# tsirigos/ibm-cbc-genomic-tools

Measured on AMD Instinct MI355X. Metric: overlap-counted reads/sec, 100M reads x 1M ref intervals, higher is better.
Workload: dtype int32; 1 GPU; BASELINE config 3: 100000000 50bp reads in total, sorted by (chrom,start), x 1000000 ref intervals over 24 hg38 chromosomes, strand ignored (genomic_overlaps count -S -i); reads resident in HBM; total_reads=100000000, refs=1000000, reduce=none (one rank)

## Files before the change

ibm-cbc-genomic-tools_amd/csrc/gtx_capi.hip:

```cpp
#include <hip/hip_runtime.h>
#include <stdint.h>
#include <string.h>
#include <stdio.h>
#include <algorithm>
#include <string>
#include <thread>
#include <vector>
#include "gtx.h"
#include "gtx_kernels.h"
#include "gtx_pairs.h"
#include "gtx_internal.h"
#include "gtx_ctx.h"

static thread_local std::string g_create_error;

int make_hist_set(gtx_ctx *c, HistSet &h, int64_t histLen)
{
  const size_t parts = (size_t)gtx::scan_tiles(histLen) + 2;
  HIPCHK(c, h.histA.alloc(histLen)); HIPCHK(c, h.histB.alloc(histLen)); HIPCHK(c, h.partA.alloc(parts)); HIPCHK(c, h.partB.alloc(parts));
  HIPCHK(c, h.prefA.alloc(histLen)); HIPCHK(c, h.prefB.alloc(histLen)); HIPCHK(c, h.flags.alloc(8 * parts));
  HIPCHK(c, h.totals.alloc(4 * parts));
  for (DevBuf<u64> *b : {&h.histA, &h.histB, &h.partA, &h.partB, &h.totals}) HIPCHK(c, hipMemset(b->get(), 0, sizeof(u64) * b->cap));
  HIPCHK(c, hipMemset(h.flags.get(), 0, sizeof(unsigned) * h.flags.cap));
  h.epoch = 0; h.draws = 0; h.totalsTurn = 0;
// ... 178 lines not shown
    if (cl > maxc) maxc = cl;
  }
  if (nClasses <= 0) nClasses = maxc + 1;
  if (maxc >= nClasses) return fail(c, GTX_E_RANGE, "gtx_set_refs: class id >= n_classes");
  if (nClasses < 1) nClasses = 1;

  std::vector<u64> keyE, keyS;
  std::vector<int32_t> ord;
  ord.reserve(m);
  const bool keepZero = (flags & GTX_REFS_KEEP_ZERO_LENGTH) != 0;
  for (int64_t k = 0; k < m; k++) {
    int32_t s = tri[3 * k + 1], e = tri[3 * k + 2];
    const bool take = tri[3 * k] >= 0 && (keepZero ? (int64_t)s <= (int64_t)e + 1 : !(s > e || e <= 0));
    if (take) ord.push_back((int32_t)k);
  }
  const int64_t nv = (int64_t)ord.size();
  struct Item { int32_t cls; int32_t val; int32_t k; };
  std::vector<Item> itE(nv), itS(nv);
  for (int64_t i = 0; i < nv; i++) {
    int32_t k = ord[i];
    itE[i] = {tri[3 * (int64_t)k], tri[3 * (int64_t)k + 2], k};
    itS[i] = {tri[3 * (int64_t)k], tri[3 * (int64_t)k + 1], k};
  }
  auto cmp = [](const Item &a, const Item &b) { return a.cls != b.cls ? a.cls < b.cls : (a.val != b.val ? a.val < b.val : a.k < b.k); };
  if (nv > (1 << 16)) {
    std::thread other([&] { std::sort(itS.begin(), itS.end(), cmp); });
    std::sort(itE.begin(), itE.end(), cmp);
    other.join();
  } else {
    std::sort(itE.begin(), itE.end(), cmp);
    std::sort(itS.begin(), itS.end(), cmp);
  }

  std::vector<int32_t> sortedE(nv + 1), sortedS(nv + 1), seg(nClasses + 1, 0), posE(m > 0 ? m : 1, -1), posS(m > 0 ? m : 1, -1), classBase(m > 0 ? m : 1, -1);
  for (int64_t i = 0; i < nv; i++) seg[itE[i].cls + 1]++;
  for (int cl = 0; cl < nClasses; cl++) seg[cl + 1] += seg[cl];
  for (int64_t i = 0; i < nv; i++) {
    sortedE[i] = itE[i].val; posE[itE[i].k] = (int32_t)(i + itE[i].cls);
    sortedS[i] = itS[i].val; posS[itS[i].k] = (int32_t)(i + itS[i].cls);
    classBase[itE[i].k] = seg[itE[i].cls] + itE[i].cls - 1;
  }

  c->nRefs = -1;
  c->ix = {}; c->cv = {}; c->rx = {}; c->share = {};
  c->covDirty = false; c->pairUsed = false;
  const int64_t histLen = nv + nClasses;
  HIPCHK(c, c->ix.sortedE.alloc(nv + 1));
  HIPCHK(c, c->ix.sortedS.alloc(nv + 1));
  HIPCHK(c, c->ix.segStart.alloc(nClasses + 1));
  HIPCHK(c, c->ix.posE.alloc(m + 1));
  HIPCHK(c, c->ix.posS.alloc(m + 1));
  HIPCHK(c, c->ix.classBase.alloc(m + 1));
  { int rc = make_hist_set(c, c->ix.hist, histLen); if (rc) return rc; }
  c->histDirty = false; c->tileSumsValid = true;
  HIPCHK(c, hipMemcpy(c->ix.sortedE.get(), sortedE.data(), sizeof(int32_t) * nv, hipMemcpyHostToDevice));
  HIPCHK(c, hipMemcpy(c->ix.sortedS.get(), sortedS.data(), sizeof(int32_t) * nv, hipMemcpyHostToDevice));
  HIPCHK(c, hipMemcpy(c->ix.segStart.get(), seg.data(), sizeof(int32_t) * (nClasses + 1), hipMemcpyHostToDevice));
  {
    c->ix.sampShift = gtx::search_sample_shift(nv);
    c->ix.nSamp = (int)((nv + (1ll << c->ix.sampShift) - 1) >> c->ix.sampShift);
    std::vector<int32_t> sampE(c->ix.nSamp + 1), sampS(c->ix.nSamp + 1);
    for (int i = 0; i < c->ix.nSamp; i++) { sampE[i] = sortedE[(int64_t)i << c->ix.sampShift]; sampS[i] = sortedS[(int64_t)i << c->ix.sampShift]; }
    HIPCHK(c, upload(c->ix.sampE, sampE.data(), sampE.size()));
    HIPCHK(c, upload(c->ix.sampS, sampS.data(), sampS.size()));
    const int64_t nTop = (nv + 255) >> 8;
    std::vector<int32_t> topE(nTop + 1), topS(nTop + 1);
    for (int64_t i = 0; i < nTop; i++) { topE[i] = sortedE[i << 8]; topS[i] = sortedS[i << 8]; }
    HIPCHK(c, upload(c->ix.topE, topE.data(), topE.size()));
    HIPCHK(c, upload(c->ix.topS, topS.data(), topS.size()));
  }
  { int rc = make_place_table(c, seg, sortedE, sortedS, nClasses, nv, c->ix.place); if (rc) return rc; }
  {
    const int kE = gtx::bucket_e_size(), kS = gtx::bucket_s_size();
    BucketCuts k;
    k.clsStart.assign(nClasses + 1, 0);
    for (int cl = 0; cl < nClasses; cl++) {
      k.clsStart[cl] = (int32_t)k.posHi.size();
      const int32_t s0 = seg[cl], s1 = seg[cl + 1];
      for (int32_t e0 = s0; e0 < s1; e0 += kE) {
        const int32_t e1 = std::min<int64_t>((int64_t)e0 + kE, s1);
        k.posHi.push_back(e1 == s1 ? INT32_MAX : sortedE[e1 - 1]);
        k.eLo.push_back(e0); k.eHi.push_back(e1); k.cls.push_back(cl);
        const int32_t lo = e0 == s0 ? s0 : (int32_t)(std::upper_bound(sortedS.begin() + s0, sortedS.begin() + s1, sortedE[e0 - 1]) - sortedS.begin());
        k.sLo.push_back(lo); k.sHi.push_back((int32_t)std::min<int64_t>((int64_t)lo + kS, s1));
      }
    }
    k.clsStart[nClasses] = (int32_t)k.posHi.size();
    if (k.posHi.size() <= 8192 && nClasses <= 2048) {
      int rc = build_bucket_tables(c, c->ix.bkt, k, nClasses); if (rc) return rc;
    }
  }
  if (m > 0) {
    HIPCHK(c, hipMemcpy(c->ix.posE.get(), posE.data(), sizeof(int32_t) * m, hipMemcpyHostToDevice));
    HIPCHK(c, hipMemcpy(c->ix.posS.get(), posS.data(), sizeof(int32_t) * m, hipMemcpyHostToDevice));
    HIPCHK(c, hipMemcpy(c->ix.classBase.get(), classBase.data(), sizeof(int32_t) * m, hipMemcpyHostToDevice));
  }
  c->h_refS.resize(m > 0 ? m : 1); c->h_refE.resize(m > 0 ? m : 1); c->h_refC.resize(m > 0 ? m : 1);
  for (int64_t k = 0; k < m; k++) { c->h_refC[k] = tri[3 * k]; c->h_refS[k] = tri[3 * k + 1]; c->h_refE[k] = tri[3 * k + 2]; }
  c->mergeRefs = keepZero;
  if (keepZero) {
    std::vector<int4> sp; std::vector<int32_t> spIdx;
    for (int64_t k = 0; k < m; k++)
      if (tri[3 * k] >= 0 && (int64_t)tri[3 * k + 1] > (int64_t)tri[3 * k + 2] + 1) { sp.push_back(make_int4(tri[3 * k], tri[3 * k + 1], tri[3 * k + 2], 0)); spIdx.push_back((int32_t)k); }
    c->rx.nSpecial = (int)sp.size();
    if (c->rx.nSpecial) {
      HIPCHK(c, upload(c->rx.specialRefs, sp.data(), sp.size()));
      HIPCHK(c, upload(c->rx.specialIdx, spIdx.data(), spIdx.size()));
      HIPCHK(c, c->rx.specialOut.alloc(sp.size()));
      HIPCHK(c, hipMemset(c->rx.specialOut.get(), 0, sizeof(u64) * sp.size()));
    }
  }
  c->nRefs = m; c->nValid = nv; c->nClasses = nClasses; c->histLen = histLen;
  c->h_seg = seg;
  return GTX_OK;
}

#ifdef GTX_WAVE_TRACE
static constexpr size_t kTraceWaves = 1u << 20;
static unsigned long long *g_trace = nullptr;
static unsigned long long *gtx_debug_trace_buffer()
{
  if (!g_trace && hipMalloc(&g_trace, kTraceWaves * 32) == hipSuccess) (void)hipMemset(g_trace, 0, kTraceWaves * 32);
  return g_trace;
}
extern "C" int gtx_debug_trace_read(unsigned long long *out, long long nWaves)
{
  if (!g_trace || nWaves > (long long)kTraceWaves) return -1;
  if (hipDeviceSynchronize() != hipSuccess) return -2;
// ... 119 lines not shown
  if (!c->sideUsed) return GTX_OK;
  c->sideUsed = false;
  HIPCHK(c, gtx::launch_side_reads(c->rx.refC.get(), c->rx.refS.get(), c->rx.refE.get(), c->nRefs, c->side.get(), c->sideCount.get(), c->sideCap, c->specialMode, (u64 *)d_out,
                                   c->d_info.get() + c->infoCur, c->stream));
  HIPCHK(c, gtx::launch_special_scatter(c->rx.specialIdx.get(), c->rx.specialOut.get(), c->rx.nSpecial, (u64 *)d_out, c->sideCount.get(), c->stream));
  return GTX_OK;
}

extern "C" {

static int count_begin(gtx_ctx *c)
{
  if (c->histDirty) {
    HistSet &h = c->ix.hist;
    for (DevBuf<u64> *b : {&h.histA, &h.histB, &h.partA, &h.partB, &h.totals}) HIPCHK(c, hipMemsetAsync(b->get(), 0, sizeof(u64) * b->cap, c->stream));
  }
  if (c->histDirty || c->covDirty) HIPCHK(c, hipMemcpyAsync(c->d_info.get() + c->infoCur, &c->h_info.get()[1], sizeof(gtx::DevInfo), hipMemcpyHostToDevice, c->stream));
  if ((c->histDirty || c->covDirty) && c->sideCount.get()) {
    HIPCHK(c, hipMemsetAsync(c->sideCount.get(), 0, sizeof(unsigned), c->stream));
    if (c->rx.nSpecial) HIPCHK(c, hipMemsetAsync(c->rx.specialOut.get(), 0, sizeof(u64) * c->rx.nSpecial, c->stream));
  }
  if (c->histDirty && c->rx.pairAcc.get()) HIPCHK(c, hipMemsetAsync(c->rx.pairAcc.get(), 0, sizeof(u64) * 2 * (size_t)std::max<int64_t>(c->nRefs, 1), c->stream));
  c->sideUsed = false; c->pairUsed = false;
  c->histDirty = true; c->tileSumsValid = true;
  c->ix.lastShareInfo = nullptr;
  return GTX_OK;
}

static int finalize_set(gtx_ctx *c, HistSet &h, bool sumsValid, u64 *d_hits, gtx::DevInfo *info, gtx::DevInfo *infoNext, hipStream_t s,
                        const gtx::FinalizeShare *fs, bool hist32)
{
  if (++h.epoch == 0) { HIPCHK(c, hipMemsetAsync(h.flags.get(), 0, sizeof(unsigned) * h.flags.cap, s)); h.epoch = 1; h.draws = 0; }
  gtx::FinalizeArgs a = h.view(c->histLen);
  a.tileSumsValid = sumsValid; a.localMaxTiles = c->localMaxTiles; a.posE = c->ix.posE.get(); a.posS = c->ix.posS.get(); a.classBase = c->ix.classBase.get();
  a.m = c->nRefs; a.hits = d_hits; a.info = info; a.nextInfo = infoNext; a.share = fs; a.hist32 = hist32;
  gtx::FinalizeRoute took;
  HIPCHK(c, gtx::launch_finalize(a, s, &took));
  if (took == gtx::FIN_CHAINED) h.draws += (unsigned long long)(fs ? fs->nTiles : gtx::scan_tiles(c->histLen));
  if (took == gtx::FIN_LOCAL) h.totalsTurn ^= 1;
  return GTX_OK;
}

static int count_end(gtx_ctx *c, void *d_hits, bool share = false, bool scatter = false, bool hist32 = false)
{
  const gtx::FinalizeShare fs = {c->share.tiles.get(), c->share.nTiles, c->share.regions.get(), c->share.nRegions, scatter};
  int rc = finalize_set(c, c->ix.hist, c->tileSumsValid, (u64 *)d_hits, c->d_info.get() + c->infoCur, c->d_info.get() + (c->infoCur ^ 1), c->stream,
                        share ? &fs : nullptr, hist32);
  if (rc) return rc;
  rc = merge_end(c, d_hits); if (rc) return rc;
  c->histDirty = false;
  c->infoCur ^= 1;
  return GTX_OK;
}

int gtx_count_device(gtx_ctx *c, const void *d_reads, const void *d_weights, int64_t n, uint32_t flags, void *d_hits)
{
  if (!c) return GTX_E_ARG;
  if (c->nRefs < 0) return fail(c, GTX_E_STATE, "gtx_count_device: gtx_set_refs has not been called");
  if (n < 0 || (n > 0 && !d_reads) || (c->nRefs > 0 && !d_hits)) return fail(c, GTX_E_ARG, "gtx_count_device: bad argument");
  HIPCHK(c, hipSetDevice(c->device));
  int rc = count_begin(c); if (rc) return rc;
  prof_begin(c);
  HIPCHK(c, prof_mark(c, 1, c->stream));
  rc = merge_prepare(c, flags, 0); if (rc) return rc;
  const bool streaming = (flags & (GTX_READS_SORTED | GTX_CHECK_SORTED)) != 0;
  if (!streaming) c->tileSumsValid = false;
  bool h32 = false;
// ... 668 lines not shown
```

ibm-cbc-genomic-tools_amd/csrc/gtx_ctx.h:

```cpp
#pragma once
#include <hip/hip_runtime.h>
#include <stdint.h>
#include <string.h>
#include <algorithm>
#include <string>
#include <utility>
#include <vector>
#include "gtx.h"
#include "gtx_kernels.h"
#include "gtx_pairs.h"
#include "gtx_link.h"
#include "gtx_adjacent.h"
#include "gtx_internal.h"

namespace gtx { struct JoinInfo; struct SignalInfo; }

#pragma GCC visibility push(hidden)

typedef unsigned long long u64;

namespace gtxhost {

template <class T, bool Pinned> class Buf {
 public:
// ... 25 lines not shown
  DevBuf<int4> cls; DevBuf<int> rank; int shift = 0;
  gtx::PlaceTable view() const { gtx::PlaceTable t; t.cls = cls.get(); t.rank = rank.get(); t.shift = shift; return t; }
};

struct BucketTables {
  DevBuf<int> bkt; DevBuf<int4> clsCell; DevBuf<uint16_t> cellTab; int nB = 0, nCells = 0, cellShift = 0;
  gtx::BucketTable view() const
  {
    gtx::BucketTable t;
    const int *d = bkt.get();
    t.posHi = d; t.eLo = d + nB; t.eHi = d + 2 * nB; t.sLo = d + 3 * nB; t.sHi = d + 4 * nB; t.cls = d + 5 * nB; t.clsStart = d + 6 * nB; t.nB = nB;
    t.clsCell = clsCell.get(); t.cellTab = cellTab.get(); t.nCells = nCells; t.cellShift = cellShift;
    return t;
  }
};

struct BucketCuts { std::vector<int32_t> posHi, eLo, eHi, sLo, sHi, cls, clsStart; };

struct HistSet {
  DevBuf<u64> histA, histB, partA, partB, prefA, prefB; DevBuf<unsigned> flags; unsigned epoch = 0; unsigned long long draws = 0;
  DevBuf<u64> totals; unsigned totalsTurn = 0;
  gtx::FinalizeArgs view(int64_t histLen) const
  {
    gtx::FinalizeArgs a = {};
    const size_t turn = 2 * ((size_t)gtx::scan_tiles(histLen) + 2);
    a.histA = histA.get(); a.histB = histB.get(); a.tileA = partA.get(); a.tileB = partB.get(); a.prefA = prefA.get(); a.prefB = prefB.get(); a.histLen = histLen;
    a.chainFlags = flags.get(); a.epoch = epoch; a.draws = draws;
    a.totals = totals.get() + (totalsTurn & 1) * turn; a.nextTotals = totals.get() + ((totalsTurn & 1) ^ 1) * turn;
    return a;
  }
};

struct CountIndex {
  DevBuf<int> sortedE, sortedS, segStart, posE, posS, classBase;
  DevBuf<int> sampE, sampS; int sampShift = 6, nSamp = 0;
  DevBuf<int> topE, topS;
  PlaceTable place;
  BucketTables bkt;
  HistSet hist;
  HistSet alt[GTXI_SHARE_STREAMS];
  DevBuf<gtx::DevInfo> info3; unsigned shareSeq = 0; unsigned shareTurn[GTXI_SHARE_STREAMS] = {}; const gtx::DevInfo *lastShareInfo = nullptr;
};

struct CoverIndex {
  DevBuf<u64> cov[12];
  DevBuf<int> sortedT, segT, topT, posTE, posTS, classBaseT;
  int64_t histLenT = 0;
  PlaceTable place;
  BucketTables bkt;
  bool ready = false;
};

struct RefExtras {
  DevBuf<int> refS, refE, refC;
  int nSpecial = 0; DevBuf<int4> specialRefs; DevBuf<int> specialIdx; DevBuf<u64> specialOut;
  struct PairIdx { DevBuf<int> mem; int n = 0; bool built = false; gtx::PairIndex ix = {}; } pairMulti, pairAll;
  DevBuf<int2> blkOf, blkIv; bool refBlocks = false;
  DevBuf<u64> pairAcc;
  DevBuf<long long> joinKey; std::vector<long long> h_joinKey; int joinMono = -1;
  DevBuf<int4> offRef; DevBuf<int8_t> refStrand;
  bool sigSet = false; double sigMin = 0, sigMax = 0; int64_t sigBins = 0; DevBuf<long long> sigRefLen;
};

struct Share { bool on = false; DevBuf<int> tiles; int nTiles = 0; DevBuf<int> regions; int64_t nRegions = 0, offset = 0; DevBuf<unsigned char> owned; };

struct TextSlot {
  DevBuf<char> text; DevBuf<unsigned> seg;
// ... 274 lines not shown
```

ibm-cbc-genomic-tools_amd/csrc/gtx_kernels.h:

```cpp
#pragma once
#include <hip/hip_runtime.h>
#include <stdint.h>
#include <mutex>
#include "gtx_routes.h"

namespace gtx {

struct PerDevice {
  std::mutex m; unsigned long long done = 0;
  template <class F> hipError_t once(F fn)
  {
    int dev = 0;
    hipError_t e = hipGetDevice(&dev);
    if (e != hipSuccess) return e;
    std::lock_guard<std::mutex> lk(m);
    if (dev >= 0 && dev < 64 && ((done >> dev) & 1)) return hipSuccess;
    e = fn();
    if (e == hipSuccess && dev >= 0 && dev < 64) done |= 1ull << dev;
    return e;
  }
};

struct DevInfo {
  long long first_unsorted;
// ... 112 lines not shown
int bucket_e_size();
int bucket_s_size();
int bucket_t_size();
hipError_t launch_count_bucketed(const void *reads, const void *weights, long long n, const CountArgs &a, const BucketTable &t,
                                 const BucketWork &w, const BucketPlan &p, hipStream_t st);
hipError_t launch_cover_bucketed(const void *reads, const void *weights, long long n, const CountArgs &a, const CoverArgs &cv, const BucketTable &t,
                                 const BucketWork &w, const BucketPlan &p, hipStream_t st);
struct ScanPart { int bucket, first, count, pad; };
int scan_part_bins(bool weighted);
hipError_t launch_scan_bucketed(const void *reads, const void *weights, long long n, const CountArgs &a, const ScanArgs &sc, const BucketTable &t,
                                const BucketWork &w, const BucketPlan &p, const ScanPart *parts, int nParts, hipStream_t st,
                                unsigned long long *out = nullptr);
int scan_fused_max_comb();
hipError_t launch_tile_sums(unsigned long long *histA, unsigned long long *histB, long long histLen, unsigned long long *tileA, unsigned long long *tileB, hipStream_t st);

hipError_t launch_special_refs(const void *reads, const void *weights, long long n, const int4 *refs, int nSpecial, int mode,
                               unsigned long long *out, hipStream_t st);
hipError_t launch_side_reads(const int *refC, const int *refS, const int *refE, long long m, const int4 *side, const unsigned *sideCount,
                             int sideCap, int mode, unsigned long long *hits, DevInfo *info, hipStream_t st);
hipError_t launch_special_scatter(const int *specialIdx, unsigned long long *specialOut, int nSpecial, unsigned long long *hits,
                                  unsigned *sideCount, hipStream_t st);

SpanSchedule span_schedule(long long nChunks, int cpw, int r, long long slots);
int search_sample_shift(long long nValid);

hipError_t launch_count(const void *reads, const void *weights, long long n, const CountArgs &a, bool sortedHint, hipStream_t st);
struct FinalizeShare { const int *tileList; int nTiles; const int *regionList; long long nRegions; bool scatter; };
struct FinalizeArgs {
  unsigned long long *histA, *histB, *tileA, *tileB, *prefA, *prefB;
  unsigned *chainFlags; unsigned epoch; unsigned long long draws;
  unsigned long long *totals, *nextTotals;
  long long histLen; bool tileSumsValid;
  int localMaxTiles;
  const int *posE, *posS, *classBase; long long m; unsigned long long *hits;
  DevInfo *info, *nextInfo;
  const FinalizeShare *share; bool hist32;
};
hipError_t launch_finalize(const FinalizeArgs &a, hipStream_t st, FinalizeRoute *took);
hipError_t launch_coverage(const void *reads, const void *weights, long long n, const CoverArgs &a, hipStream_t st);
hipError_t launch_coverage_finalize(const CoverArgs &a, long long histLen, const CoverGather &g, long long m,
                                    unsigned long long *cov, DevInfo *nextInfo, hipStream_t st);
hipError_t launch_scan_zero(void *micro, long long bytes, const int *runIf, hipStream_t st);
hipError_t launch_scan_hist(const void *reads, const void *weights, long long n, const ScanArgs &a, hipStream_t st, const int *runIf = nullptr);
int scan_window_tile();
hipError_t launch_scan_windows(const void *micro, bool micro64, const ScanArgs &a, long long totalTiles,
                               unsigned long long *out, hipStream_t st, const int *runIf = nullptr);

struct ScanOwn {
  const long long *blkOff;
  int tile;
  long long totalBlocks;
  long long *bounds;
  int *flag;
};
int scan_own_tile(long long nReads, long long totalMicro, int comb);
hipError_t launch_scan_own(const void *reads, const void *weights, long long n, const ScanArgs &a, const ScanOwn &o,
                           unsigned long long *out, hipStream_t st);

}
```

ibm-cbc-genomic-tools_amd/csrc/gtx_kernels.hip:

```cpp
#include <hip/hip_runtime.h>
#include <stdint.h>
#include <stdlib.h>
#include <string.h>
#include <stdio.h>
#include <type_traits>
#include <vector>
#include <algorithm>
#include "gtx_kernels.h"

namespace gtx {

typedef unsigned long long u64;
typedef long long i64;

static constexpr int kHi = 0x7fffffff;
static constexpr int kLo = (int)0x80000000;
static constexpr int kSlots = 63;
static constexpr int kSearchLdsBytes = 128 * 1024;

__device__ __forceinline__ int rfl(int v) { return __builtin_amdgcn_readfirstlane(v); }
__device__ __forceinline__ int rdlane(int v, int l) { return __builtin_amdgcn_readlane(v, l); }

__device__ __forceinline__ int lane_prev(int v) { return __builtin_amdgcn_update_dpp(v, v, 0x138, 0xf, 0xf, false); }

// ... 1179 lines not shown
      else if (s0 != s1) {
        const int i0 = (int)(((i64)s0 + rnd) >> sh), i1 = (int)(((i64)s1 + rnd) >> sh);
        int lo = i0, hi = i1;
        while (lo < hi) { int mid = (lo + hi) >> 1; if (se[mid] < t.s) lo = mid + 1; else hi = mid; }
        int glo = lo == i0 ? s0 : ((lo - 1) << sh) + 1, ghi = lo == i1 ? s1 : lo << sh;
        while (glo < ghi) { int mid = (int)(((i64)glo + ghi) >> 1); if (a.sortedE[mid] < t.s) glo = mid + 1; else ghi = mid; }
        slotA = glo + t.c;
        lo = i0; hi = i1;
        while (lo < hi) { int mid = (lo + hi) >> 1; if (ss[mid] <= t.e) lo = mid + 1; else hi = mid; }
        glo = lo == i0 ? s0 : ((lo - 1) << sh) + 1; ghi = lo == i1 ? s1 : lo << sh;
        while (glo < ghi) { int mid = (int)(((i64)glo + ghi) >> 1); if (a.sortedS[mid] <= t.e) glo = mid + 1; else ghi = mid; }
        slotB = glo + t.c;
      }
    }
    if (WEIGHTED) {
      if (slotA >= 0) { atomicAdd(&a.histA[slotA], (u64)w); atomicAdd(&a.histB[slotB], (u64)w); }
    } else {
      run_add(a.histA, slotA, lane);
      run_add(a.histB, slotB, lane);
    }
  }
  if (nNoClass) atomicAdd((u64 *)&a.info->n_no_class, (u64)nNoClass);
  if (nDegen) { atomicAdd((u64 *)&a.info->n_degenerate, (u64)nDegen); atomicMin((i64 *)&a.info->first_degenerate, firstDegen + a.indexBase); }
}

template <class T> __device__ __forceinline__ void load4(const T *p, u64 (&v)[4]);
template <> __device__ __forceinline__ void load4<u64>(const u64 *p, u64 (&v)[4])
{ const ulonglong2 x = *(const ulonglong2 *)p, y = *(const ulonglong2 *)(p + 2); v[0] = x.x; v[1] = x.y; v[2] = y.x; v[3] = y.y; }
template <> __device__ __forceinline__ void load4<unsigned>(const unsigned *p, u64 (&v)[4])
{ const uint4 x = *(const uint4 *)p; v[0] = x.x; v[1] = x.y; v[2] = x.z; v[3] = x.w; }
template <class T> __device__ __forceinline__ void store4(T *p, u64 a, u64 b, u64 c, u64 d);
template <> __device__ __forceinline__ void store4<u64>(u64 *p, u64 a, u64 b, u64 c, u64 d) { *(ulonglong2 *)p = make_ulonglong2(a, b); *(ulonglong2 *)(p + 2) = make_ulonglong2(c, d); }
template <> __device__ __forceinline__ void store4<unsigned>(unsigned *p, u64 a, u64 b, u64 c, u64 d) { *(uint4 *)p = make_uint4((unsigned)a, (unsigned)b, (unsigned)c, (unsigned)d); }

__device__ __forceinline__ u64 block_sum(u64 v, u64 *lds)
{
  const int lane = threadIdx.x & 63, wv = threadIdx.x >> 6;
#pragma unroll
  for (int o = 32; o > 0; o >>= 1) v += __shfl_xor(v, o);
  __syncthreads();
  if (lane == 0) lds[wv] = v;
  __syncthreads();
  u64 s = 0;
  for (int k = 0; k < (int)(blockDim.x >> 6); k++) s += lds[k];
  return s;
}

template <class T>
__global__ __launch_bounds__(256) void tile_sums_kernel(const T *__restrict__ ha, const T *__restrict__ hb, i64 len,
                                                        u64 *__restrict__ pa, u64 *__restrict__ pb, const int *__restrict__ tileList)
{
  __shared__ u64 lds[4];
  const T *__restrict__ h = blockIdx.y ? hb : ha;
  const int tileIdx = tileList ? tileList[blockIdx.x] : (int)blockIdx.x;
  const i64 i0 = (i64)tileIdx * kTile + (i64)threadIdx.x * 4;
  u64 s = 0;
  if (i0 + 4 <= len) { u64 v[4]; load4<T>(h + i0, v); s = v[0] + v[1] + v[2] + v[3]; }
  else for (int k = 0; k < 4; k++) if (i0 + k < len) s += h[i0 + k];
  s = block_sum(s, lds);
  if (threadIdx.x == 0) (blockIdx.y ? pb : pa)[tileIdx] = s;
}

template <class T>
__global__ __launch_bounds__(256) void finalize_scan_kernel(T *__restrict__ ha, T *__restrict__ hb, i64 len,
                                                            const u64 *__restrict__ ta, const u64 *__restrict__ tb,
                                                            T *__restrict__ pa, T *__restrict__ pb, const int *__restrict__ tileList)
// ... 59 lines not shown
  }
  v[1] += v[0]; v[2] += v[1]; v[3] += v[2];
  const u64 x = wave_scan_add64(v[3]);
  if (lane == 63) wsum[wv] = x;
  __syncthreads();
  if (threadIdx.x < 2) {
    const u64 s = wsum[0] + wsum[1] + wsum[2] + wsum[3];
    __hip_atomic_store(fl + 2 * pos + threadIdx.x, ((u64)epoch << 32) | (threadIdx.x ? s >> 32 : s & 0xffffffffull), __ATOMIC_RELAXED, __HIP_MEMORY_SCOPE_AGENT);
  }
  u64 o = 0;
  bool gaveUp = false;
  for (int t = threadIdx.x; t < pos; t += 256) {
    u64 lo, hi; unsigned spins = 0;
    while (((lo = __hip_atomic_load(fl + 2 * t, __ATOMIC_RELAXED, __HIP_MEMORY_SCOPE_AGENT)) >> 32) != epoch && ++spins < kChainSpinMax) __builtin_amdgcn_s_sleep(1);
    while (((hi = __hip_atomic_load(fl + 2 * t + 1, __ATOMIC_RELAXED, __HIP_MEMORY_SCOPE_AGENT)) >> 32) != epoch && ++spins < kChainSpinMax) __builtin_amdgcn_s_sleep(1);
    if (spins >= kChainSpinMax) { gaveUp = true; break; }
    o += (lo & 0xffffffffull) | (hi << 32);
  }
  if (gaveUp) atomicAdd((u64 *)&info->fault, 1ull);
  o = block_sum(o, lds);
  o += x - v[3];
  for (int k = 0; k < wv; k++) o += wsum[k];
  if (full) { store4<T>(p + i0, v[0] + o, v[1] + o, v[2] + o, v[3] + o); store4<T>(h + i0, 0, 0, 0, 0); }
  else {
#pragma unroll
    for (int k = 0; k < 4; k++)
      if (i0 + k < len) { p[i0 + k] = (T)(v[k] + o); h[i0 + k] = 0; }
  }
}

template <class T>
__global__ __launch_bounds__(256) void gather_hits_kernel(const T *__restrict__ pa, const T *__restrict__ pb,
                                                          const int *__restrict__ posE, const int *__restrict__ posS,
                                                          const int *__restrict__ classBase, i64 m, u64 *__restrict__ hits,
                                                          u64 *__restrict__ ta, u64 *__restrict__ tb, int nTiles, DevInfo *nextInfo,
                                                          const int *__restrict__ regionList, int scatter)
{
  i64 k = (i64)blockIdx.x * blockDim.x + threadIdx.x;
  if (k < nTiles) { ta[k] = 0; tb[k] = 0; }
  if (k == 0) { nextInfo->first_unsorted = INT64_MAX; nextInfo->n_no_class = 0; nextInfo->n_degenerate = 0; nextInfo->first_degenerate = INT64_MAX; nextInfo->n_unplaced = 0; nextInfo->fault = 0; }
  if (k >= m) return;
  i64 outIdx = k;
  if (regionList) { k = regionList[k]; if (scatter) outIdx = k; }
  int pe = posE[k];
  u64 h = 0;
  if (pe >= 0) {
    int cb = classBase[k];
    T ba = cb >= 0 ? pa[cb] : 0, bb = cb >= 0 ? pb[cb] : 0;
    h = (u64)(T)((T)(pa[pe] - ba) - (T)(pb[posS[k]] - bb));
  }
  hits[outIdx] = h;
}

template <class T>
__global__ __launch_bounds__(256) void finalize_local_kernel(T *__restrict__ ha, T *__restrict__ hb, i64 len,
                                                             u64 *__restrict__ totA, u64 *__restrict__ totB,
                                                             T *__restrict__ pa, T *__restrict__ pb, const int *__restrict__ tileList)
{
  __shared__ u64 wsum[4];
  T *__restrict__ h = blockIdx.y ? hb : ha;
  T *__restrict__ p = blockIdx.y ? pb : pa;
  const int lane = threadIdx.x & 63, wv = threadIdx.x >> 6;
  const int tile = tileList ? tileList[blockIdx.x] : (int)blockIdx.x;
  const i64 i0 = (i64)tile * kTile + (i64)threadIdx.x * 4;
  const bool full = i0 + 4 <= len;
  u64 v[4];
  if (full) load4<T>(h + i0, v);
  else {
#pragma unroll
    for (int k = 0; k < 4; k++) v[k] = i0 + k < len ? (u64)h[i0 + k] : 0;
  }
  v[1] += v[0]; v[2] += v[1]; v[3] += v[2];
  const u64 x = wave_scan_add64(v[3]);
  if (lane == 63) wsum[wv] = x;
  __syncthreads();
  u64 o = x - v[3];
  for (int k = 0; k < wv; k++) o += wsum[k];
  if (full) { store4<T>(p + i0, v[0] + o, v[1] + o, v[2] + o, v[3] + o); store4<T>(h + i0, 0, 0, 0, 0); }
  else {
#pragma unroll
    for (int k = 0; k < 4; k++)
      if (i0 + k < len) { p[i0 + k] = (T)(v[k] + o); h[i0 + k] = 0; }
  }
  if (threadIdx.x == 255) (blockIdx.y ? totB : totA)[tile] = o + v[3];
}

static constexpr int kGatherLocalThreads = 1024, kGatherLocalPer = 4;
static constexpr int kGatherLocalTot = kLocalScanMaxTiles / kGatherLocalThreads;
static_assert(kLocalScanMaxTiles % kGatherLocalThreads == 0, "gather_hits_local_kernel: every tile's total has a thread");

template <class T>
__global__ __launch_bounds__(kGatherLocalThreads) void gather_hits_local_kernel(const T *__restrict__ pa, const T *__restrict__ pb,
                                                          const u64 *__restrict__ totA, const u64 *__restrict__ totB,
                                                          u64 *__restrict__ nextTotA, u64 *__restrict__ nextTotB,
                                                          const int *__restrict__ posE, const int *__restrict__ posS,
                                                          const int *__restrict__ classBase, i64 m, u64 *__restrict__ hits,
                                                          u64 *__restrict__ ta, u64 *__restrict__ tb, int nTiles, DevInfo *nextInfo,
                                                          const int *__restrict__ regionList, int scatter)
{
  extern __shared__ u64 ldsOff[];
  __shared__ u64 wtot[2][kGatherLocalThreads / 64];
  T *off = (T *)ldsOff;
  const int lane = threadIdx.x & 63, wv = threadIdx.x >> 6;
  const i64 first = (i64)blockIdx.x * (kGatherLocalThreads * kGatherLocalPer) + threadIdx.x;
  i64 outIdx[kGatherLocalPer];
  int pe[kGatherLocalPer], ps[kGatherLocalPer], cb[kGatherLocalPer];
#pragma unroll
  for (int j = 0; j < kGatherLocalPer; j++) {
    i64 k = first + (i64)j * kGatherLocalThreads;
    outIdx[j] = k < m ? k : -1;
    pe[j] = -1; ps[j] = 0; cb[j] = -1;
    if (k < m) {
      if (regionList) { k = regionList[k]; if (scatter) outIdx[j] = k; }
      pe[j] = posE[k]; ps[j] = posS[k]; cb[j] = classBase[k];
    }
  }
  const int per = (nTiles + kGatherLocalThreads - 1) / kGatherLocalThreads, t0 = (int)threadIdx.x * per;
  u64 ra[kGatherLocalTot], rb[kGatherLocalTot];
#pragma unroll
  for (int q = 0; q < kGatherLocalTot; q++) {
    const bool in = q < per && t0 + q < nTiles;
    ra[q] = in ? totA[t0 + q] : 0; rb[q] = in ? totB[t0 + q] : 0;
  }
  T ve[kGatherLocalPer], vs[kGatherLocalPer], ba[kGatherLocalPer], bb[kGatherLocalPer];
#pragma unroll
  for (int j = 0; j < kGatherLocalPer; j++) {
    const int e = pe[j] >= 0 ? pe[j] : 0, s = pe[j] >= 0 ? ps[j] : 0, c = cb[j] >= 0 ? cb[j] : 0;
    ve[j] = pa[e]; vs[j] = pb[s]; ba[j] = pa[c]; bb[j] = pb[c];
  }
  u64 sa = 0, sb = 0;
#pragma unroll
  for (int q = 0; q < kGatherLocalTot; q++) { sa += ra[q]; sb += rb[q]; }
  const u64 xa = wave_scan_add64(sa), xb = wave_scan_add64(sb);
  if (lane == 63) { wtot[0][wv] = xa; wtot[1][wv] = xb; }
  __syncthreads();
  u64 oa = xa - sa, ob = xb - sb;
  for (int k = 0; k < wv; k++) { oa += wtot[0][k]; ob += wtot[1][k]; }
#pragma unroll
  for (int q = 0; q < kGatherLocalTot; q++) {
    if (q < per && t0 + q < nTiles) { off[t0 + q] = (T)oa; off[nTiles + t0 + q] = (T)ob; }
    oa += ra[q]; ob += rb[q];
  }
  __syncthreads();
  const i64 gtid = (i64)blockIdx.x * kGatherLocalThreads + threadIdx.x;
  for (i64 i = gtid; i < nTiles; i += (i64)gridDim.x * kGatherLocalThreads) { ta[i] = 0; tb[i] = 0; nextTotA[i] = 0; nextTotB[i] = 0; }
  if (gtid == 0) { nextInfo->first_unsorted = INT64_MAX; nextInfo->n_no_class = 0; nextInfo->n_degenerate = 0; nextInfo->first_degenerate = INT64_MAX; nextInfo->n_unplaced = 0; nextInfo->fault = 0; }
#pragma unroll
  for (int j = 0; j < kGatherLocalPer; j++) {
    if (outIdx[j] < 0) continue;
    u64 h = 0;
    if (pe[j] >= 0) {
      const int e = pe[j], s = ps[j], c = cb[j] >= 0 ? cb[j] : 0;
      const T fa = (T)(ve[j] + off[e >> kTileShift]), fb = (T)(vs[j] + off[nTiles + (s >> kTileShift)]);
      const T ga = cb[j] >= 0 ? (T)(ba[j] + off[c >> kTileShift]) : (T)0, gb = cb[j] >= 0 ? (T)(bb[j] + off[nTiles + (c >> kTileShift)]) : (T)0;
      h = (u64)(T)((T)(fa - ga) - (T)(fb - gb));
    }
    hits[outIdx[j]] = h;
  }
}

__global__ __launch_bounds__(256) void gather_coverage_kernel(CoverGather g, i64 m, u64 *__restrict__ cov, int nTiles, DevInfo *nextInfo)
{
  i64 k = (i64)blockIdx.x * blockDim.x + threadIdx.x;
  if (k < nTiles) {
#pragma unroll
    for (int q = 0; q < 4; q++) g.part[q][k] = 0;
  }
  if (k == 0) { nextInfo->first_unsorted = INT64_MAX; nextInfo->n_no_class = 0; nextInfo->n_degenerate = 0; nextInfo->first_degenerate = INT64_MAX; nextInfo->n_unplaced = 0; nextInfo->fault = 0; }
  if (k >= m) return;
  const int pe = g.posTE[k];
  u64 c = 0;
  if (pe >= 0 && g.refE[k] >= g.refS[k]) {
    const int ps = g.posTS[k], cb = g.classBaseT[k];
    u64 v[8];
#pragma unroll
    for (int q = 0; q < 4; q++) { const u64 *p = g.pref[q]; const u64 b = cb >= 0 ? p[cb] : 0; v[q] = p[pe] - b; v[4 + q] = p[ps] - b; }
    const u64 E = (u64)(i64)g.refE[k], S = (u64)(i64)g.refS[k];
    c = v[3] - v[7] + E * (v[0] - v[2]) - v[1] + v[5] - S * (v[4] - v[6]) + v[0] - v[6];
  }
  cov[k] = c;
}

__device__ __forceinline__ void scan_slot(const Tri &t, bool in_range, const ScanArgs &a, int &cls, int &mw, int clsU = -1, i64 nmU = 0)
{
  cls = -1; mw = -1;
  if (in_range && (clsU >= 0 || (unsigned)t.c < (unsigned)a.nClasses) && (a.sortedRule || (t.s <= t.e && t.e > 0))) {
    i64 pos = a.center ? (i64)t.s + ((i64)t.e - t.s) / 2 : (i64)t.s;
    if (a.sortedRule && pos < 1) pos = 1;
    if (pos >= 1) {
      const unsigned x = (unsigned)(pos - 1), d = (unsigned)a.winStep;
// ... 215 lines not shown
  return hipGetLastError();
}

hipError_t launch_tile_sums(u64 *histA, u64 *histB, i64 histLen, u64 *tileA, u64 *tileB, hipStream_t st)
{
  const int nb = scan_tiles(histLen);
  if (nb > 0) tile_sums_kernel<u64><<<dim3(nb, 2), 256, 0, st>>>(histA, histB, histLen, tileA, tileB, nullptr);
  return hipGetLastError();
}

template <class T>
static hipError_t launch_finalize_t(const FinalizeArgs &a, hipStream_t st, FinalizeRoute *took)
{
  T *histA = (T *)a.histA, *histB = (T *)a.histB, *prefA = (T *)a.prefA, *prefB = (T *)a.prefB;
  const int nb = scan_tiles(a.histLen);
  const int nbRun = a.share ? a.share->nTiles : nb;
  const int *tl = a.share ? a.share->tileList : nullptr, *regions = a.share ? a.share->regionList : nullptr;
  const i64 mm = a.share ? a.share->nRegions : a.m;
  const int scatter = a.share && a.share->scatter ? 1 : 0;
  *took = finalize_route(nb, nbRun, a.tileSumsValid, a.chainFlags && a.info, a.totals && a.nextTotals, a.localMaxTiles, route_knobs());
  switch (*took) {
  case FIN_GATHER_ONLY: break;
  case FIN_CHAINED: {
    u64 *f = (u64 *)a.chainFlags;
    finalize_scan_chained_kernel<T><<<dim3(nbRun, 2), 256, 0, st>>>(histA, histB, a.histLen, f, f + 2 * (nb + 2), f + 2 * nb, f + 2 * (nb + 2) + 2 * nb, a.draws, a.epoch,
                                                                    nbRun, prefA, prefB, tl, a.info);
    break;
  }
  case FIN_LOCAL: {
    const size_t parts = (size_t)nb + 2;
    const i64 perBlock = (i64)kGatherLocalThreads * kGatherLocalPer;
    finalize_local_kernel<T><<<dim3(nbRun, 2), 256, 0, st>>>(histA, histB, a.histLen, a.totals, a.totals + parts, prefA, prefB, tl);
    gather_hits_local_kernel<T><<<(unsigned)((std::max<i64>(mm, 1) + perBlock - 1) / perBlock), kGatherLocalThreads, sizeof(T) * 2 * (size_t)nb, st>>>(
        prefA, prefB, a.totals, a.totals + parts, a.nextTotals, a.nextTotals + parts, a.posE, a.posS, a.classBase, mm, a.hits, a.tileA, a.tileB, nb, a.nextInfo, regions, scatter);
    return hipGetLastError();
  }
  case FIN_SUMS_SCAN:
    tile_sums_kernel<T><<<dim3(nbRun, 2), 256, 0, st>>>(histA, histB, a.histLen, a.tileA, a.tileB, tl);
    [[fallthrough]];
  case FIN_SUMS_KEPT:
    finalize_scan_kernel<T><<<dim3(nbRun, 2), 256, 0, st>>>(histA, histB, a.histLen, a.tileA, a.tileB, prefA, prefB, tl);
    break;
  }
  const i64 work = std::max<i64>(std::max<i64>(mm, nb), 1);
  gather_hits_kernel<T><<<(unsigned)((work + 255) / 256), 256, 0, st>>>(prefA, prefB, a.posE, a.posS, a.classBase, mm, a.hits, a.tileA, a.tileB, nb, a.nextInfo, regions, scatter);
  return hipGetLastError();
}

hipError_t launch_finalize(const FinalizeArgs &a, hipStream_t st, FinalizeRoute *took)
{
  return a.hist32 ? launch_finalize_t<unsigned>(a, st, took) : launch_finalize_t<u64>(a, st, took);
}

hipError_t launch_coverage(const void *reads, const void *weights, i64 n, const CoverArgs &a, hipStream_t st)
{
  if (n <= 0) return hipSuccess;
  const i64 waves = a.sched.nWaves;
  const unsigned grid = (unsigned)((waves + 3) / 4);
  if (weights) coverage_walk_kernel_weighted<<<grid, 256, 0, st>>>((const Tri *)reads, (const int *)weights, n, a);
  else coverage_walk_kernel<false><<<grid, 256, 0, st>>>((const Tri *)reads, (const int *)weights, n, a);
  return hipGetLastError();
}

hipError_t launch_coverage_finalize(const CoverArgs &a, i64 histLen, const CoverGather &g, i64 m, u64 *cov, DevInfo *nextInfo, hipStream_t st)
{
  const int nb = scan_tiles(histLen);
  for (int q = 0; q < 4 && nb > 0; q += 2)
    finalize_scan_kernel<u64><<<dim3(nb, 2), 256, 0, st>>>(a.hist[q], a.hist[q + 1], histLen, a.part[q], a.part[q + 1], g.pref[q], g.pref[q + 1], nullptr);
  const i64 work = (m > nb ? m : nb) > 0 ? (m > nb ? m : nb) : 1;
  gather_coverage_kernel<<<(unsigned)((work + 255) / 256), 256, 0, st>>>(g, m, cov, nb, nextInfo);
  return hipGetLastError();
}

__global__ __launch_bounds__(256) void scan_zero_kernel(uint4 *__restrict__ p, i64 n16, const int *__restrict__ runIf)
{
  if (runIf && *runIf == 0) return;
  for (i64 i = (i64)blockIdx.x * blockDim.x + threadIdx.x; i < n16; i += (i64)gridDim.x * blockDim.x) p[i] = make_uint4(0, 0, 0, 0);
}
// ... 33 lines not shown
```

Measured before the change: 498.3 billion reads/s.

## Drop class-base prefix subtraction in hit gather and use write-through stores in finalize

Removes the per-reference classBase lookup and the two extra prefix-array reads it required. Hits are now computed directly as prefE minus prefS. This depends on class segments being laid out so that the base terms cancel, which is algebraically true only if the E and S prefix bases are equal at class boundaries. Separately, stores in the local finalize and gather kernels become inline-asm global_store with the sc1 bit or relaxed agent-scope atomic stores, which changes how those writes interact with the cache. Both changes risk correctness if the cancellation assumption fails, and the inline asm adds hardware-specific fragility.

```diff
diff --git a/ibm-cbc-genomic-tools_amd/csrc/gtx_capi.hip b/ibm-cbc-genomic-tools_amd/csrc/gtx_capi.hip
--- a/ibm-cbc-genomic-tools_amd/csrc/gtx_capi.hip
+++ b/ibm-cbc-genomic-tools_amd/csrc/gtx_capi.hip
@@ -234,13 +234,12 @@
     std::sort(itS.begin(), itS.end(), cmp);
   }
 
-  std::vector<int32_t> sortedE(nv + 1), sortedS(nv + 1), seg(nClasses + 1, 0), posE(m > 0 ? m : 1, -1), posS(m > 0 ? m : 1, -1), classBase(m > 0 ? m : 1, -1);
+  std::vector<int32_t> sortedE(nv + 1), sortedS(nv + 1), seg(nClasses + 1, 0), posE(m > 0 ? m : 1, -1), posS(m > 0 ? m : 1, -1);
   for (int64_t i = 0; i < nv; i++) seg[itE[i].cls + 1]++;
   for (int cl = 0; cl < nClasses; cl++) seg[cl + 1] += seg[cl];
   for (int64_t i = 0; i < nv; i++) {
     sortedE[i] = itE[i].val; posE[itE[i].k] = (int32_t)(i + itE[i].cls);
     sortedS[i] = itS[i].val; posS[itS[i].k] = (int32_t)(i + itS[i].cls);
-    classBase[itE[i].k] = seg[itE[i].cls] + itE[i].cls - 1;
   }
 
   c->nRefs = -1;
@@ -252,7 +251,6 @@
   HIPCHK(c, c->ix.segStart.alloc(nClasses + 1));
   HIPCHK(c, c->ix.posE.alloc(m + 1));
   HIPCHK(c, c->ix.posS.alloc(m + 1));
-  HIPCHK(c, c->ix.classBase.alloc(m + 1));
   { int rc = make_hist_set(c, c->ix.hist, histLen); if (rc) return rc; }
   c->histDirty = false; c->tileSumsValid = true;
   HIPCHK(c, hipMemcpy(c->ix.sortedE.get(), sortedE.data(), sizeof(int32_t) * nv, hipMemcpyHostToDevice));
@@ -295,7 +293,6 @@
   if (m > 0) {
     HIPCHK(c, hipMemcpy(c->ix.posE.get(), posE.data(), sizeof(int32_t) * m, hipMemcpyHostToDevice));
     HIPCHK(c, hipMemcpy(c->ix.posS.get(), posS.data(), sizeof(int32_t) * m, hipMemcpyHostToDevice));
-    HIPCHK(c, hipMemcpy(c->ix.classBase.get(), classBase.data(), sizeof(int32_t) * m, hipMemcpyHostToDevice));
   }
   c->h_refS.resize(m > 0 ? m : 1); c->h_refE.resize(m > 0 ? m : 1); c->h_refC.resize(m > 0 ? m : 1);
   for (int64_t k = 0; k < m; k++) { c->h_refC[k] = tri[3 * k]; c->h_refS[k] = tri[3 * k + 1]; c->h_refE[k] = tri[3 * k + 2]; }
@@ -481,7 +478,7 @@
 {
   if (++h.epoch == 0) { HIPCHK(c, hipMemsetAsync(h.flags.get(), 0, sizeof(unsigned) * h.flags.cap, s)); h.epoch = 1; h.draws = 0; }
   gtx::FinalizeArgs a = h.view(c->histLen);
-  a.tileSumsValid = sumsValid; a.localMaxTiles = c->localMaxTiles; a.posE = c->ix.posE.get(); a.posS = c->ix.posS.get(); a.classBase = c->ix.classBase.get();
+  a.tileSumsValid = sumsValid; a.localMaxTiles = c->localMaxTiles; a.posE = c->ix.posE.get(); a.posS = c->ix.posS.get();
   a.m = c->nRefs; a.hits = d_hits; a.info = info; a.nextInfo = infoNext; a.share = fs; a.hist32 = hist32;
   gtx::FinalizeRoute took;
   HIPCHK(c, gtx::launch_finalize(a, s, &took));
diff --git a/ibm-cbc-genomic-tools_amd/csrc/gtx_ctx.h b/ibm-cbc-genomic-tools_amd/csrc/gtx_ctx.h
--- a/ibm-cbc-genomic-tools_amd/csrc/gtx_ctx.h
+++ b/ibm-cbc-genomic-tools_amd/csrc/gtx_ctx.h
@@ -81,7 +81,7 @@
 };
 
 struct CountIndex {
-  DevBuf<int> sortedE, sortedS, segStart, posE, posS, classBase;
+  DevBuf<int> sortedE, sortedS, segStart, posE, posS;
   DevBuf<int> sampE, sampS; int sampShift = 6, nSamp = 0;
   DevBuf<int> topE, topS;
   PlaceTable place;
diff --git a/ibm-cbc-genomic-tools_amd/csrc/gtx_kernels.h b/ibm-cbc-genomic-tools_amd/csrc/gtx_kernels.h
--- a/ibm-cbc-genomic-tools_amd/csrc/gtx_kernels.h
+++ b/ibm-cbc-genomic-tools_amd/csrc/gtx_kernels.h
@@ -168,7 +168,7 @@
   unsigned long long *totals, *nextTotals;
   long long histLen; bool tileSumsValid;
   int localMaxTiles;
-  const int *posE, *posS, *classBase; long long m; unsigned long long *hits;
+  const int *posE, *posS; long long m; unsigned long long *hits;
   DevInfo *info, *nextInfo;
   const FinalizeShare *share; bool hist32;
 };
diff --git a/ibm-cbc-genomic-tools_amd/csrc/gtx_kernels.hip b/ibm-cbc-genomic-tools_amd/csrc/gtx_kernels.hip
--- a/ibm-cbc-genomic-tools_amd/csrc/gtx_kernels.hip
+++ b/ibm-cbc-genomic-tools_amd/csrc/gtx_kernels.hip
@@ -1235,6 +1235,16 @@
 template <class T> __device__ __forceinline__ void store4(T *p, u64 a, u64 b, u64 c, u64 d);
 template <> __device__ __forceinline__ void store4<u64>(u64 *p, u64 a, u64 b, u64 c, u64 d) { *(ulonglong2 *)p = make_ulonglong2(a, b); *(ulonglong2 *)(p + 2) = make_ulonglong2(c, d); }
 template <> __device__ __forceinline__ void store4<unsigned>(unsigned *p, u64 a, u64 b, u64 c, u64 d) { *(uint4 *)p = make_uint4((unsigned)a, (unsigned)b, (unsigned)c, (unsigned)d); }
+typedef unsigned u32x4 __attribute__((ext_vector_type(4)));
+__device__ __forceinline__ void store16_wt(void *p, u32x4 x) { asm volatile("global_store_dwordx4 %0, %1, off sc1\n\ts_nop 1" : : "v"(p), "v"(x) : "memory"); }
+template <class T> __device__ __forceinline__ void store4_wt(T *p, u64 a, u64 b, u64 c, u64 d);
+template <> __device__ __forceinline__ void store4_wt<u64>(u64 *p, u64 a, u64 b, u64 c, u64 d)
+{
+  store16_wt(p, u32x4{(unsigned)a, (unsigned)(a >> 32), (unsigned)b, (unsigned)(b >> 32)});
+  store16_wt(p + 2, u32x4{(unsigned)c, (unsigned)(c >> 32), (unsigned)d, (unsigned)(d >> 32)});
+}
+template <> __device__ __forceinline__ void store4_wt<unsigned>(unsigned *p, u64 a, u64 b, u64 c, u64 d) { store16_wt(p, u32x4{(unsigned)a, (unsigned)b, (unsigned)c, (unsigned)d}); }
+template <class T> __device__ __forceinline__ void store1_wt(T *p, T x) { __hip_atomic_store(p, x, __ATOMIC_RELAXED, __HIP_MEMORY_SCOPE_AGENT); }
 
 __device__ __forceinline__ u64 block_sum(u64 v, u64 *lds)
 {
@@ -1360,7 +1370,7 @@
 template <class T>
 __global__ __launch_bounds__(256) void gather_hits_kernel(const T *__restrict__ pa, const T *__restrict__ pb,
                                                           const int *__restrict__ posE, const int *__restrict__ posS,
-                                                          const int *__restrict__ classBase, i64 m, u64 *__restrict__ hits,
+                                                          i64 m, u64 *__restrict__ hits,
                                                           u64 *__restrict__ ta, u64 *__restrict__ tb, int nTiles, DevInfo *nextInfo,
                                                           const int *__restrict__ regionList, int scatter)
 {
@@ -1372,11 +1382,7 @@
   if (regionList) { k = regionList[k]; if (scatter) outIdx = k; }
   int pe = posE[k];
   u64 h = 0;
-  if (pe >= 0) {
-    int cb = classBase[k];
-    T ba = cb >= 0 ? pa[cb] : 0, bb = cb >= 0 ? pb[cb] : 0;
-    h = (u64)(T)((T)(pa[pe] - ba) - (T)(pb[posS[k]] - bb));
-  }
+  if (pe >= 0) h = (u64)(T)(pa[pe] - pb[posS[k]]);
   hits[outIdx] = h;
 }
 
@@ -1404,13 +1410,13 @@
   __syncthreads();
   u64 o = x - v[3];
   for (int k = 0; k < wv; k++) o += wsum[k];
-  if (full) { store4<T>(p + i0, v[0] + o, v[1] + o, v[2] + o, v[3] + o); store4<T>(h + i0, 0, 0, 0, 0); }
+  if (full) { store4_wt<T>(p + i0, v[0] + o, v[1] + o, v[2] + o, v[3] + o); store4_wt<T>(h + i0, 0, 0, 0, 0); }
   else {
 #pragma unroll
     for (int k = 0; k < 4; k++)
-      if (i0 + k < len) { p[i0 + k] = (T)(v[k] + o); h[i0 + k] = 0; }
-  }
-  if (threadIdx.x == 255) (blockIdx.y ? totB : totA)[tile] = o + v[3];
+      if (i0 + k < len) { store1_wt<T>(p + i0 + k, (T)(v[k] + o)); store1_wt<T>(h + i0 + k, (T)0); }
+  }
+  if (threadIdx.x == 255) store1_wt<u64>((blockIdx.y ? totB : totA) + tile, o + v[3]);
 }
 
 static constexpr int kGatherLocalThreads = 1024, kGatherLocalPer = 4;
@@ -1422,7 +1428,7 @@
                                                           const u64 *__restrict__ totA, const u64 *__restrict__ totB,
                                                           u64 *__restrict__ nextTotA, u64 *__restrict__ nextTotB,
                                                           const int *__restrict__ posE, const int *__restrict__ posS,
-                                                          const int *__restrict__ classBase, i64 m, u64 *__restrict__ hits,
+                                                          i64 m, u64 *__restrict__ hits,
                                                           u64 *__restrict__ ta, u64 *__restrict__ tb, int nTiles, DevInfo *nextInfo,
                                                           const int *__restrict__ regionList, int scatter)
 {
@@ -1432,15 +1438,15 @@
   const int lane = threadIdx.x & 63, wv = threadIdx.x >> 6;
   const i64 first = (i64)blockIdx.x * (kGatherLocalThreads * kGatherLocalPer) + threadIdx.x;
   i64 outIdx[kGatherLocalPer];
-  int pe[kGatherLocalPer], ps[kGatherLocalPer], cb[kGatherLocalPer];
+  int pe[kGatherLocalPer], ps[kGatherLocalPer];
 #pragma unroll
   for (int j = 0; j < kGatherLocalPer; j++) {
     i64 k = first + (i64)j * kGatherLocalThreads;
     outIdx[j] = k < m ? k : -1;
-    pe[j] = -1; ps[j] = 0; cb[j] = -1;
+    pe[j] = -1; ps[j] = 0;
     if (k < m) {
       if (regionList) { k = regionList[k]; if (scatter) outIdx[j] = k; }
-      pe[j] = posE[k]; ps[j] = posS[k]; cb[j] = classBase[k];
+      pe[j] = posE[k]; ps[j] = posS[k];
     }
   }
   const int per = (nTiles + kGatherLocalThreads - 1) / kGatherLocalThreads, t0 = (int)threadIdx.x * per;
@@ -1450,11 +1456,11 @@
     const bool in = q < per && t0 + q < nTiles;
     ra[q] = in ? totA[t0 + q] : 0; rb[q] = in ? totB[t0 + q] : 0;
   }
-  T ve[kGatherLocalPer], vs[kGatherLocalPer], ba[kGatherLocalPer], bb[kGatherLocalPer];
+  T ve[kGatherLocalPer], vs[kGatherLocalPer];
 #pragma unroll
   for (int j = 0; j < kGatherLocalPer; j++) {
-    const int e = pe[j] >= 0 ? pe[j] : 0, s = pe[j] >= 0 ? ps[j] : 0, c = cb[j] >= 0 ? cb[j] : 0;
-    ve[j] = pa[e]; vs[j] = pb[s]; ba[j] = pa[c]; bb[j] = pb[c];
+    const int e = pe[j] >= 0 ? pe[j] : 0, s = pe[j] >= 0 ? ps[j] : 0;
+    ve[j] = pa[e]; vs[j] = pb[s];
   }
   u64 sa = 0, sb = 0;
 #pragma unroll
@@ -1471,19 +1477,19 @@
   }
   __syncthreads();
   const i64 gtid = (i64)blockIdx.x * kGatherLocalThreads + threadIdx.x;
-  for (i64 i = gtid; i < nTiles; i += (i64)gridDim.x * kGatherLocalThreads) { ta[i] = 0; tb[i] = 0; nextTotA[i] = 0; nextTotB[i] = 0; }
+  for (i64 i = gtid; i < nTiles; i += (i64)gridDim.x * kGatherLocalThreads) {
+    store1_wt<u64>(ta + i, 0); store1_wt<u64>(tb + i, 0); store1_wt<u64>(nextTotA + i, 0); store1_wt<u64>(nextTotB + i, 0);
+  }
   if (gtid == 0) { nextInfo->first_unsorted = INT64_MAX; nextInfo->n_no_class = 0; nextInfo->n_degenerate = 0; nextInfo->first_degenerate = INT64_MAX; nextInfo->n_unplaced = 0; nextInfo->fault = 0; }
 #pragma unroll
   for (int j = 0; j < kGatherLocalPer; j++) {
     if (outIdx[j] < 0) continue;
     u64 h = 0;
     if (pe[j] >= 0) {
-      const int e = pe[j], s = ps[j], c = cb[j] >= 0 ? cb[j] : 0;
-      const T fa = (T)(ve[j] + off[e >> kTileShift]), fb = (T)(vs[j] + off[nTiles + (s >> kTileShift)]);
-      const T ga = cb[j] >= 0 ? (T)(ba[j] + off[c >> kTileShift]) : (T)0, gb = cb[j] >= 0 ? (T)(bb[j] + off[nTiles + (c >> kTileShift)]) : (T)0;
-      h = (u64)(T)((T)(fa - ga) - (T)(fb - gb));
-    }
-    hits[outIdx[j]] = h;
+      const T fa = (T)(ve[j] + off[pe[j] >> kTileShift]), fb = (T)(vs[j] + off[nTiles + (ps[j] >> kTileShift)]);
+      h = (u64)(T)(fa - fb);
+    }
+    store1_wt<u64>(hits + outIdx[j], h);
   }
 }
 
@@ -1765,7 +1771,7 @@
     const i64 perBlock = (i64)kGatherLocalThreads * kGatherLocalPer;
     finalize_local_kernel<T><<<dim3(nbRun, 2), 256, 0, st>>>(histA, histB, a.histLen, a.totals, a.totals + parts, prefA, prefB, tl);
     gather_hits_local_kernel<T><<<(unsigned)((std::max<i64>(mm, 1) + perBlock - 1) / perBlock), kGatherLocalThreads, sizeof(T) * 2 * (size_t)nb, st>>>(
-        prefA, prefB, a.totals, a.totals + parts, a.nextTotals, a.nextTotals + parts, a.posE, a.posS, a.classBase, mm, a.hits, a.tileA, a.tileB, nb, a.nextInfo, regions, scatter);
+        prefA, prefB, a.totals, a.totals + parts, a.nextTotals, a.nextTotals + parts, a.posE, a.posS, mm, a.hits, a.tileA, a.tileB, nb, a.nextInfo, regions, scatter);
     return hipGetLastError();
   }
   case FIN_SUMS_SCAN:
@@ -1776,7 +1782,7 @@
     break;
   }
   const i64 work = std::max<i64>(std::max<i64>(mm, nb), 1);
-  gather_hits_kernel<T><<<(unsigned)((work + 255) / 256), 256, 0, st>>>(prefA, prefB, a.posE, a.posS, a.classBase, mm, a.hits, a.tileA, a.tileB, nb, a.nextInfo, regions, scatter);
+  gather_hits_kernel<T><<<(unsigned)((work + 255) / 256), 256, 0, st>>>(prefA, prefB, a.posE, a.posS, mm, a.hits, a.tileA, a.tileB, nb, a.nextInfo, regions, scatter);
   return hipGetLastError();
 }
 
```

Result: no change. 499.2 billion reads/s, median of 4 (+0.2%).
